# haberdashPI/SignalOperators.jl

Hardware: AMD Instinct MI355X
Metric: frames/sec sink() 44.1kHz 8ch Mix+Filt+Resample; achieved HBM GB/s (higher is better)
Workload: dtype f64

## Files before the change

signaloperators.jl_amd/csrc/executor.cpp:

```cpp
#include "plan_impl.h"

namespace so {

static inline int carrier_vec_ok(const DCarrier& c, int64_t V) {
    if (!std::getenv("SIGOPS_STRICT_ALIGN")) return (uintptr_t)c.base % (c.dtype == SO_F64 ? 8 : 4) == 0;
    return ((uintptr_t)c.base % 16 == 0) && (c.cstride % V == 0);
}

static hipError_t h2d_small(void* dst, const void* src, size_t bytes) {
    constexpr size_t kPiece = 16 * 1024;
    if (bytes < 2 * kPiece || bytes > (1u << 20)) return hipMemcpy(dst, src, bytes, hipMemcpyHostToDevice);
    for (size_t off = 0; off < bytes; off += kPiece) {
        const hipError_t e = hipMemcpy((char*)dst + off, (const char*)src + off, std::min(kPiece, bytes - off), hipMemcpyHostToDevice);
        if (e != hipSuccess) return e;
    }
    return hipSuccess;
}

static void upload_tables(Plan* P) {
    std::vector<Buf>& bufs = P->bufs;
    auto up = [&](int buf, const auto& v, size_t at = 0) {
        HIPCHECK(h2d_small((char*)bufs[buf].d + at, v.data(), v.size() * sizeof(*v.data())));
    };
    auto alloc_up = [](auto*& d, const auto& v) {
// ... 470 lines not shown
}
static RsGlobalTables global_tables(Plan* P, const Stage& S) {
    return RsGlobalTables{(const RsCtl*)P->bufs[S.ctl_buf].d, (const DCarrier*)P->bufs[S.car_buf].d, P->d_ops, P->d_leaves};
}
static void set_rsos_fixup(RsFixup& F, Plan* P, const Stage& S, const RsosItem& I) {
    F.g = I.g;
    F.tab = I.tab;
    F.jend = I.jend;
    F.jrel = (const int*)P->bufs[S.rsos_jrel_buf].d;
    F.taps = S.rsos_taps;
    F.cf = S.groups[0];
    F.gsrc = I.gsrc;
    F.y = I.y;
}
static void arm_bad(void* words, size_t n, hipStream_t st) { HIPCHECK((hipError_t)launch_fill_u32(words, n, 0x7f7f7f7fu, st)); }

static std::vector<long long> read_trace(const long long* d_trace, size_t trace_n, hipStream_t st, long long& t0) {
    std::vector<long long> tr(trace_n);
    HIPCHECK(hipStreamSynchronize(st));
    HIPCHECK(hipMemcpy(tr.data(), d_trace, trace_n * 8, hipMemcpyDeviceToHost));
    t0 = 0;
    for (size_t i = 0; i < trace_n; ++i)
        if (tr[i] && (!t0 || tr[i] < t0)) t0 = tr[i];
    return tr;
}
static void dump_rs_trace(const long long* d_trace, size_t trace_n, const RsPeriodic& rp, hipStream_t st) {
    long long t0;
    const std::vector<long long> tr = read_trace(d_trace, trace_n, st, t0);
    for (int w = 0; w < rp.nwaves; ++w)
        for (int it = 0; it < kRsTraceIters; ++it) {
            const long long* q = &tr[((size_t)w * kRsTraceIters + it) * kRsTraceStamps];
            if (!q[0]) continue;
            std::fprintf(stderr, "[rs-trace] %s w%02d it%02d", w < rp.ncompute ? "C" : "L", w, it);
            for (int k = 0; k < kRsTraceStamps; ++k) std::fprintf(stderr, " %lld", q[k] ? q[k] - t0 : -1);
            std::fprintf(stderr, "\n");
        }
}
static void dump_rsos_trace(const long long* d_trace, size_t trace_n, const RsSos& rs, hipStream_t st) {
    long long t0;
    const std::vector<long long> tr = read_trace(d_trace, trace_n, st, t0);
    const bool counters = std::atoi(std::getenv("SIGOPS_RSOS_TRACE")) == 2;
    for (int w = 0; w < rs.nwaves; ++w)
        for (int it = 0; it < (counters ? 5 : kRsosTraceIters); ++it) {
            const long long* q = &tr[((size_t)w * kRsosTraceIters + it) * 8];
            if (counters) {
                bool any = false;
                for (int k = 0; k < 8; ++k) any = any || q[k];
                if (!any) continue;
                std::fprintf(stderr, "[rsos-count] w%02d row%d", w, it);
                for (int k = 0; k < 8; ++k) std::fprintf(stderr, " %lld", q[k] - 1);
            } else {
                if (!q[0] && !q[2]) continue;
                std::fprintf(stderr, "[rsos-trace] %s w%02d it%02d", w == 0 ? "C" : (w & 3) == 0 ? "L" : "Y", w, it);
                for (int k = 0; k < 8; ++k) std::fprintf(stderr, " %lld", q[k] ? q[k] - t0 : -1);
            }
            std::fprintf(stderr, "\n");
        }
}


static int run_pointwise(Plan* P, const Step& s, void* outp, hipStream_t st) {
    const PwStep& w = P->pw[s.idx];
    if (w.nblocks <= 0) return 0;
    static const int il_scalar = std::getenv("SIGOPS_K1_ILSCALAR") ? 1 : 0;
    OutView ov{};
    if (w.out_buf >= 0) {
        const Buf& b = P->bufs[w.out_buf];
        ov = OutView{b.d, 1, b.pitch, b.dtype, il_scalar};
    } else if (P->out.is_device) {
        ov = OutView{outp, P->out.frame_stride, P->out.chan_stride, P->out.dtype, il_scalar};
    } else {
        const Buf& b = P->bufs[P->out_stage_buf];
// ... 75 lines not shown
        RsSos rs = S.rs;
        rs.out_pitch = out.pitch;
        rs.out_f32 = P->nodes[S.node].dtype == SO_F32;
        rs.f32m = 0;
        rs.sring = 0;
        rs.mats = (const double*)P->bufs[S.rsos_mats_buf].d;
        rs.bad = poison ? (int32_t*)P->bufs[B.bad_buf].d + B.bad_off[m] : nullptr;
        rs.err = kernel_error_word(P);
        I.g = rs;
        I.tab = (const double*)P->bufs[S.rsos_tab_buf].d;
        I.jend = (const int*)P->bufs[S.rsos_jend_buf].d;
        I.y = out.d - (size_t)S.rs.store_lo * (rs.out_f32 ? 4 : 8);
        I.gsrc = global_tables(P, S);
        std::memset(&fix[m], 0, sizeof fix[m]);
        set_rsos_fixup(fix[m], P, S, I);
        maxch = std::max(maxch, (int)rs.nch);
        out_f32 = rs.out_f32;
    }
    if (B.host.size() != nm || std::memcmp(B.host.data(), items.data(), nm * sizeof(RsosItem)) != 0 ||
        std::memcmp(B.fhost.data(), fix.data(), nm * sizeof(RsFixup)) != 0) {
        B.host = items;
        B.fhost = fix;
        HIPCHECK(hipMemcpyAsync(P->bufs[B.items_buf].d, B.host.data(), nm * sizeof(RsosItem), hipMemcpyHostToDevice, st));
        HIPCHECK(hipMemcpyAsync(P->bufs[B.fix_buf].d, B.fhost.data(), nm * sizeof(RsFixup), hipMemcpyHostToDevice, st));
    }
    if (poison) arm_bad(P->bufs[B.bad_buf].d, P->bufs[B.bad_buf].bytes / 4, st);
    if (launch_rsos_batch((const RsosItem*)P->bufs[B.items_buf].d, (int)nm, B.gpm, items[0].g, st) != 0)
        fail(SO_ERR_RUNTIME, "internal: no batched one-pass IIR instantiation for this geometry");
    int nl = 1;
    if (poison) nl += launch_rsos_fixup_batch((const RsFixup*)P->bufs[B.fix_buf].d, (int)nm, maxch, out_f32, st);
    return nl;
}

static int run_sample_at(Plan* P, const Step& s, void* outp, hipStream_t st) {
    const Stage& S = P->stages[s.idx];
    const Node& N = P->nodes[S.node];
    const int xdt = P->nodes[N.kids[0]].dtype;
    const View in = stage_in(P, S, N.nch, xdt), out = stage_out(P, s.idx, outp);
    SampleAtArgs a{};
    a.x = in.d;
    a.xcs = in.pitch;
    a.xfs = S.x_fstride;
    a.N = S.in_frames;
    a.x_f32 = xdt == SO_F32;
    if (S.pos_array_node >= 0) {
// ... 51 lines not shown
    a.x = in.d;
    a.xcs = in.pitch;
    a.xfs = S.x_fstride;
    a.x_f32 = xdt == SO_F32;
    a.y = (double*)out.d;
    a.ycs = out.pitch;
    a.n = S.need;
    a.nch = N.nch;
    a.tot_pitch = cumsum_totals(S.need);
    a.tot = S.aux_buf >= 0 ? (double*)P->bufs[S.aux_buf].d : nullptr;
    const int nl = launch_cumsum(a, st);
    if (nl < 0) fail(SO_ERR_UNSUPPORTED, "Cumsum: more than 65535 channels, or 2^31 chunks of 16384 frames and more, are not lowered");
    return nl;
}

static int run_rsos_fused(Plan* P, const Stage& S, const SosGeom& g, const View& out, hipStream_t st) {
    const Node& N = P->nodes[S.node];
    const Stage& S3 = P->stages[S.rsos_src];
    RsSos rs = S.rs;
    rs.out_pitch = out.pitch;
    rs.out_f32 = g.out_dtype == SO_F32 || N.dtype == SO_F32;
    if (rs.f32m && rs.out_f32) rs.ring32 = 1;
    else rs.f32m = 0;
    rs.sring = rs.f32m && (rs.fuse == 1 || rs.fuse == 2) && !std::getenv("SIGOPS_RSOS_NO_SRING") ? 1 : 0;
    char* const yk = out.d - (size_t)S.rs.store_lo * (rs.out_f32 ? 4 : 8);
    rs.store_lo = S.rs.store_lo + g.store_lo;
    rs.mats = (const double*)P->bufs[S.rsos_mats_buf].d;
    rs.bad = nullptr;
    if (S.bad_buf >= 0 && rs.nranges >= 1 && !std::getenv("SIGOPS_SOS_NOPOISON")) {
        rs.bad = (int32_t*)P->bufs[S.bad_buf].d;
        arm_bad(rs.bad, (size_t)N.nch, st);
    }
    rs.err = kernel_error_word(P);
    static long long* d_rtrace = nullptr;
    static int rtrace_seen = 0;
    const char* const rtrace_skip = std::getenv("SIGOPS_RSOS_TRACE_SKIP");
    const bool rtracing = std::getenv("SIGOPS_RSOS_TRACE") != nullptr && rtrace_seen++ >= (rtrace_skip ? std::atoi(rtrace_skip) : 0);
    const size_t rtrace_n = (size_t)16 * kRsosTraceIters * 8;
    if (rtracing) {
        if (!d_rtrace) HIPCHECK(hipMalloc(&d_rtrace, rtrace_n * 8));
        HIPCHECK(hipMemsetAsync(d_rtrace, 0, rtrace_n * 8, st));
        rs.trace = d_rtrace;
    }
    const double* rtab = (const double*)P->bufs[S.rsos_tab_buf >= 0 ? S.rsos_tab_buf : S3.tab_buf].d;
    const int* rjend = (const int*)P->bufs[S.rsos_jend_buf >= 0 ? S.rsos_jend_buf : S3.jend_buf].d;
    if (launch_rsos(rtab, rjend, rs, yk, global_tables(P, S3), S.rsos_grid, st) != 0)
        fail(SO_ERR_RUNTIME, "internal: no fused resampler + IIR instantiation for this geometry");
    if (rtracing) dump_rsos_trace(d_rtrace, rtrace_n, rs, st);
    int nl = 1;
    if (rs.bad && S.rsos_jrel_buf >= 0 && !std::getenv("SIGOPS_RSOS_NO_FIXUP")) {
        RsFixup fx{};
        set_rsos_fixup(fx, P, S, RsosItem{rs, rtab, rjend, yk, global_tables(P, S3)});
        nl += launch_rsos_fixup(fx, st);
    } else if (rs.bad) {
        SosGeom pg = g;
        pg.n = rs.n_out;
        pg.chunk = rs.pr * rs.L;
        pg.nchunks = rs.nranges;
        pg.store_lo = rs.store_lo;
        pg.bad = rs.bad;
        nl += launch_sos_poison(yk, pg, st);
    }
    return nl;
}

static int run_sos(Plan* P, const Step& s, void* outp, hipStream_t st) {
    const Stage& S = P->stages[s.idx];
    const Node& N = P->nodes[S.node];
    const size_t esz = dsize(N.dtype);
    const View in = stage_in(P, S, N.nch, N.dtype), out = stage_out(P, s.idx, outp);
    SosGeom g = S.sg;
    g.in_pitch = in.pitch;
    g.out_pitch = out.pitch;
    g.store_lo = s.idx == P->alias_stage ? P->alias_skip : 0;
    if (s.idx == P->alias_stage && P->alias_narrow) g.out_dtype = SO_F32;
    g.align_rows = S.pre_stage < 0 && !std::getenv("SIGOPS_SOS_NOALIGN");
    g.bad = nullptr;
    if (S.rsos_src >= 0) return run_rsos_fused(P, S, g, out, st);
    if (S.bad_buf >= 0 && S.pre_stage < 0 && !S.onepass && !S.xscan && !g.exact && !std::getenv("SIGOPS_SOS_NOPOISON")) {
        g.bad = (int32_t*)P->bufs[S.bad_buf].d;
        arm_bad(g.bad, (size_t)N.nch, st);
    }
// ... 500 lines not shown
```

signaloperators.jl_amd/csrc/k_exact.hip:

```cpp
#include "kcommon.h"
#include "kstage.h"

namespace so {

constexpr int kFixThreads = 256;
constexpr int kFixSeg = 1024;
constexpr int kFixIn = 6144;
constexpr int kFixAhead = 64;

template <typename TO>
__device__ __forceinline__ void rsos_fixup_body(const RsFixup& fx) {
    const RsSos& g = fx.g;
    const int ch = blockIdx.y;
    if (ch >= g.nch) return;
    const int r = g.bad[ch];
    if (r < 0 || r >= g.nranges) return;
    TO* const y = (TO*)fx.y + (int64_t)ch * g.out_pitch;
    const int64_t prL = g.pr * g.L;
    const double nan = __longlong_as_double(0x7ff8000000000000ll);
    {
        int64_t f0 = (int64_t)(r + 1) * prL;
        if (f0 < g.store_lo) f0 = g.store_lo;
        for (int64_t f = f0 + (int64_t)blockIdx.x * kFixThreads + threadIdx.x; f < g.n_out; f += (int64_t)gridDim.x * kFixThreads) y[f] = (TO)nan;
    }
    if (blockIdx.x != 0) return;
    __shared__ long long s_first;
    __shared__ double xin[kFixIn];
    __shared__ double xs[kFixSeg];
    __shared__ double ys[kFixAhead + 16];
    const int tid = threadIdx.x;
    const int64_t lo = max((int64_t)r * prL, g.store_lo), hi = min((int64_t)(r + 1) * prL, g.n_out);
// ... 64 lines not shown
                    if (!isfinite(v) || (sizeof(TO) == 4 && !isfinite((double)(float)v))) {
                        s_bad = m;
                        break;
                    }
                    ys[m - bs] = v;
                }
            }
        }
        __syncthreads();
        if (s_bad >= 0) break;
        seg = se;
    }
    const int64_t mb = s_bad;
    if (mb < 0) return;
    for (int64_t m = max(bs, lo) + tid; m < mb; m += kFixThreads) y[m] = (TO)ys[m - bs];
}

template <typename TO>
__global__ __launch_bounds__(kFixThreads) void k_rsos_fixup(RsFixup fx) {
    rsos_fixup_body<TO>(fx);
}
template <typename TO>
__global__ __launch_bounds__(kFixThreads) void k_rsos_fixup_batch(const RsFixup* __restrict__ items) {
    const RsFixup* fx = items + blockIdx.z;
    const int ch = blockIdx.y;
    if (ch >= fx->g.nch) return;
    const int r = fx->g.bad[ch];
    if (r < 0 || r >= fx->g.nranges) return;
    const RsFixup F = *fx;
    rsos_fixup_body<TO>(F);
// ... 73 lines not shown
```

signaloperators.jl_amd/csrc/k_rsos.hip:

```cpp
#include "kcommon.h"
#include "kstage.h"

#ifndef SO_RSOS_ONLY_KS
#define SO_RSOS_ONLY_KS -1
#endif
#ifndef SO_RSOS_ONLY_F32
#define SO_RSOS_ONLY_F32 0
#endif
#ifndef SO_RSOS_ONLY_NW
#define SO_RSOS_ONLY_NW 0
#endif

namespace so {

typedef double v4d __attribute__((ext_vector_type(4)));
typedef float v4f __attribute__((ext_vector_type(4)));

#define SO_LDS __attribute__((address_space(3)))
__device__ __forceinline__ int flag_ld(uint32_t a) { return *(const volatile SO_LDS int*)(uintptr_t)a; }
__device__ __forceinline__ void flag_st(uint32_t a, int v) { *(volatile SO_LDS int*)(uintptr_t)a = v; }
#define SO_SPIN_PAUSE(spins, sleep, limit)                         \
    do {                                                           \
        if (++(spins) > (limit)) rsos_wait_failed(sh);             \
        if ((sleep) == 1) __builtin_amdgcn_s_sleep(1);             \
// ... 215 lines not shown
    uint32_t SO_GLB* const e = (uint32_t SO_GLB*)rfl64((int64_t)(uintptr_t)sh->g.err);
    if (e == nullptr) __builtin_trap();
    if ((threadIdx.x & 63) == 0) __hip_atomic_store((uint32_t*)e, 1u, __ATOMIC_RELAXED, __HIP_MEMORY_SCOPE_SYSTEM);
    __threadfence_system();
    asm volatile("s_waitcnt vmcnt(0) lgkmcnt(0)" ::: "memory");
    __builtin_amdgcn_endpgm();
}

#ifndef SO_RSOS_TRACE
#define SO_RSOS_TRACE 0
#endif
__device__ __forceinline__ void rsos_stamp(long long* trace, int wave, int it, int k, int it0 = 400) {
    if constexpr (!SO_RSOS_TRACE) return;
    if (trace != nullptr && blockIdx.x == 0 && (threadIdx.x & 63) == 0 && it >= it0 && it < it0 + kRsosTraceIters)
        ((long long SO_GLB*)trace)[(wave * kRsosTraceIters + (it - it0)) * 8 + k] = clock64();
}

#ifndef SO_RSOS_COUNT
#define SO_RSOS_COUNT 0
#endif
__device__ __forceinline__ void rsos_count_out(long long* trace, int wave, int row, int k, long long v) {
    if constexpr (!SO_RSOS_COUNT) return;
    if (trace != nullptr && blockIdx.x == 0) ((long long SO_GLB*)trace)[((wave * kRsosTraceIters) + row) * 8 + k] = v + 1;
}

struct RsosLds {
    SO_LDS double *taps, *ring, *gtab;
    volatile SO_LDS double *xs, *ss;
    volatile SO_LDS double* xh;
};
// ... 682 lines not shown
        if (issued >= NK) break;
        SO_SPIN_PAUSE(spins, 2, 1 << 22);
        if constexpr (SO_RSOS_COUNT) ++cnt_idle;
    }
    __builtin_amdgcn_s_setprio(0);
    if constexpr (SO_RSOS_COUNT) {
        if (lane == 0) {
            rsos_count_out(trace, wave, 0, 0, cnt_idle);
            rsos_count_out(trace, wave, 0, 4, clock64() - cyc0);
        }
    }
}

typedef double v2d_a8 __attribute__((ext_vector_type(2), aligned(8)));

__device__ __forceinline__ bool rsos_wproj_group(const RsosShared& sh, int64_t G) {
    const RsSos& g = sh.g;
    const DCarrier& C0 = sh.ctl.car[0];
    if (!g.wproj || g.src32 || g.arr2 || g.fuse < -1 || g.ct < 8) return false;
    if (!(C0.base != nullptr && C0.vec_ok && C0.dtype == SO_F64) || (C0.df & 1)) return false;
    const int64_t ncg = g.nch / g.ct;
    const int64_t r0 = (G / ncg) * g.rgs, r1 = r0 + g.rgs - 1;
    if (r1 >= g.nranges || r0 * g.pr < g.wp) return false;
    if (g.store_lo > r0 * g.pr * g.L) return false;
    const int64_t lo_ok = C0.a > 0 ? C0.a : 0, hi_ok = C0.b < g.n_in ? C0.b : g.n_in;
    const int64_t f0 = (r0 * g.pr - g.wp) * g.M + g.wj0, f1 = (r1 * g.pr - g.wp) * g.M + g.wj0 + g.wk;
    return f0 >= lo_ok && f1 <= hi_ok;
}

template <int NY>
__device__ __attribute__((noinline)) void rsos_wproj_y(RsosShared* sh_, double* dyn, int64_t G_, int yi_) {
    constexpr int NX = 2 * NY + 1;
    const int lane = threadIdx.x & 63;
    SO_LDS RsosShared* const sh = (SO_LDS RsosShared*)rsos_lds_ptr(sh_);
    const int64_t G = rfl64(G_);
    const int yi = uni(yi_);
    const SO_LDS RsSos& g = sh->g;
    const RsosLds l = rsos_carve(dyn, uni(g.cyc) > 0 ? 0 : uni(g.ngroups) * uni(g.ks) * 64, uni(g.rpitch), NX, rsos_nss(NY));
    const uint32_t fl_base = (uint32_t)(uintptr_t)sh->flags;
    const int ct = uni(g.ct), K = uni(g.wk);
    const int npairs = (K + 7) >> 3;
    const int c0 = (int)((int64_t)yi * npairs / NY), c1 = (int)((int64_t)(yi + 1) * npairs / NY);
    const double SO_GLB* const V = (const double SO_GLB*)rfl64((int64_t)(uintptr_t)g.mats) + 14 * 64 + lane;
    const SO_LDS DCarrier& C0 = sh->ctl.car[0];
    const int64_t ncg = uni(g.nch) / ct;
    const int gq = lane >> 4, n16 = lane & 15;
    const int64_t r = (G / ncg) * uni(g.rgs) + n16 / ct;
    const int64_t f0 = (r * rfl64(g.pr) - uni(g.wp)) * rfl64(g.M) + uni(g.wj0);
    const double SO_GLB* const row = (const double SO_GLB*)rfl64((int64_t)(uintptr_t)C0.base) +
                                     ((int64_t)((int)(G % ncg) * ct + n16 % ct) * rfl64(C0.cstride) + rfl64(C0.df) + f0 + 2 * gq);
    v4d acc = v4d{0.0, 0.0, 0.0, 0.0};
    auto mm = [&](const double (&a)[16], const v2d (&b)[8]) __attribute__((always_inline)) {
#pragma unroll
        for (int i = 0; i < 8; ++i) {
            acc = __builtin_amdgcn_mfma_f64_16x16x4f64(a[2 * i], b[i][0], acc, 0, 0, 0);
            acc = __builtin_amdgcn_mfma_f64_16x16x4f64(a[2 * i + 1], b[i][1], acc, 0, 0, 0);
        }
    };
    auto load = [&](int c, double (&a)[16], v2d (&b)[8]) __attribute__((always_inline)) {
        const double SO_GLB* const vp = V + (size_t)c * 128;
        const double SO_GLB* const rp = row + (size_t)c * 8;
#pragma unroll
        for (int i = 0; i < 8; ++i) {
            a[2 * i] = vp[i * 128];
            a[2 * i + 1] = vp[i * 128 + 64];
            b[i] = *(const v2d_a8 SO_GLB*)(rp + 8 * i);
        }
    };
    double aA[16], aB[16];
    v2d bA[8], bB[8];
    const int c1f = min(c1, K >> 3);
    const int nfull = c1f > c0 ? (c1f - c0) >> 3 : 0;
    if (nfull > 0) {
        load(c0, aA, bA);
        for (int n = 0; n < nfull; n += 2) {
            const int c = c0 + 8 * n;
            if (n + 1 < nfull) load(c + 8, aB, bB);
            mm(aA, bA);
            if (n + 2 < nfull) load(c + 16, aA, bA);
            if (n + 1 < nfull) mm(aB, bB);
        }
    }
    {
        const int c = c0 + 8 * nfull;
#pragma unroll
        for (int i = 0; i < 8; ++i) {
            const int cc = c + i;
            aA[2 * i] = aA[2 * i + 1] = 0.0;
            bA[i] = v2d{0.0, 0.0};
            if (cc < c1) {
                aA[2 * i] = V[(size_t)(2 * cc) * 64];
                aA[2 * i + 1] = V[(size_t)(2 * cc + 1) * 64];
                const int f = 8 * cc + 2 * gq;
                if (f + 1 < K) bA[i] = *(const v2d_a8 SO_GLB*)(row + 8 * cc);
                else if (f < K) bA[i][0] = row[8 * cc];
            }
        }
        mm(aA, bA);
    }
#pragma unroll
    for (int v = 0; v < 3; ++v) l.ss[(1 + yi) * 192 + v * 64 + lane] = acc[v];
    flag_st(fl_base + 4 * (kRsosFlagWp + yi), 1);
}

template <int NY>
__device__ __attribute__((noinline)) void rsos_wproj_chain(RsosShared* sh_, double* dyn, int64_t G_) {
    constexpr int NX = 2 * NY + 1;
    const int lane = threadIdx.x & 63;
    SO_LDS RsosShared* const sh = (SO_LDS RsosShared*)rsos_lds_ptr(sh_);
    const int64_t G = rfl64(G_);
    const SO_LDS RsSos& g = sh->g;
    const RsosLds l = rsos_carve(dyn, uni(g.cyc) > 0 ? 0 : uni(g.ngroups) * uni(g.ks) * 64, uni(g.rpitch), NX, rsos_nss(NY));
    const uint32_t fl_base = (uint32_t)(uintptr_t)sh->flags;
    const int ct = uni(g.ct), fuse = uni(g.fuse);
    const int gq = lane >> 4, n16 = lane & 15;
    double s[3] = {0.0, 0.0, 0.0};
    if (fuse >= 0) {
        const SO_LDS DCarrier& C0 = sh->ctl.car[0];
        const DLeaf leaf0 = leaf_uniform(sh_->ctl.leaves[min(kCtlLeaves - 1, max(0, uni(C0.slot_leaf[0])))]);
        const int64_t ncg = uni(g.nch) / ct;
        const int64_t r = (G / ncg) * uni(g.rgs) + n16 / ct;
        const int64_t f0 = (r * rfl64(g.pr) - uni(g.wp)) * rfl64(g.M) + uni(g.wj0);
        const double2 sc = rsos_sine_at(f0 + leaf0.df + 1, leaf0.v0, leaf0.v1, leaf0.v2, leaf0.flag);
        const double SO_GLB* const W = (const double SO_GLB*)rfl64((int64_t)(uintptr_t)g.mats) + 14 * 64 + (size_t)((uni(g.wk) + 7) >> 3) * 128;
#pragma unroll
        for (int v = 0; v < 3; ++v) {
            const double t = fma(sc.y, W[gq + 4 * v], sc.x * W[16 + gq + 4 * v]);
            s[v] = fuse == 2 ? -t : t;
        }
    }
    int spins = 0;
    for (;;) {
        const int f = lane < NY ? flag_ld(fl_base + 4 * (kRsosFlagWp + lane)) : 1;
        if (wave_min(f, NY) >= 1) break;
        SO_SPIN_PAUSE(spins, 1, 1 << 22);
    }
#pragma unroll
    for (int yi = 0; yi < NY; ++yi)
#pragma unroll
        for (int v = 0; v < 3; ++v) s[v] += l.ss[(1 + yi) * 192 + v * 64 + lane];
#pragma unroll
    for (int v = 0; v < 3; ++v) l.ss[v * 64 + lane] = s[v];
}
// ... 477 lines not shown
    const int ru = g.ct < 8 ? g.ct : 8;
    for (int64_t G = G0; G < ngrp; G += Gstep) {
        __syncthreads();
        if (threadIdx.x < kRsosFlags) sh.flags[threadIdx.x] = 0;
        if (threadIdx.x < 192) ss[threadIdx.x] = 0.0;
        if (threadIdx.x == 0) {
            const bool pj = NW != 16 && NW != 17 && rsos_wproj_group(sh, G);
            sh.proj = pj ? 1 : 0;
            sh.wpe = pj ? 0 : g.wp;
            if (pj) sh.flags[kRsosFlagSseq] = -1;
        }
        __syncthreads();
        const bool proj = sh.proj != 0;
        if (wave == 0) {
            if (!(g.debug & 64)) {
                if (proj) rsos_wproj_chain<NY>(&sh, lds_raw, G);
                const int nk = (g.debug & 131072) ? 3 : (2 * g.nsec + 3) / 4;
                if (nk <= 1) rsos_chain<NY, 1>(&sh, lds_raw, G);
                else if (nk == 2) rsos_chain<NY, 2>(&sh, lds_raw, G);
                else rsos_chain<NY, 3>(&sh, lds_raw, G);
            }
        } else if (NW == 16 && (wave == 13 || wave == 14)) {
            if (!g.gsplit || (g.debug & 256) || g.src32) continue;
            const int q = wave - 13;
            if (g.arr2) {
                if constexpr (NL == 2) {
                    if (ru == 8) rsos_loader<NY, NL, 8, false, 0, 2, true>(&sh, lds_raw, G, q);
                    else if (ru == 4) rsos_loader<NY, NL, 4, false, 0, 2, true>(&sh, lds_raw, G, q);
                    else if (ru == 2) rsos_loader<NY, NL, 2, false, 0, 2, true>(&sh, lds_raw, G, q);
                }
            } else if (ru == 2) {
                if (g.rpitch == 770) rsos_loader<NY, NL, 2, false, 770 * 8, 2>(&sh, lds_raw, G, q);
                else if (g.rpitch == 642) rsos_loader<NY, NL, 2, false, 642 * 8, 2>(&sh, lds_raw, G, q);
                else rsos_loader<NY, NL, 2, false, 0, 2>(&sh, lds_raw, G, q);
            } else if (ru == 4) {
// ... 40 lines not shown
                else if (g.rpitch == 770) rsos_loader<NY, NL, 2, false, 770 * 8>(&sh, lds_raw, G, q);
                else if (g.rpitch == 642) rsos_loader<NY, NL, 2, false, 642 * 8>(&sh, lds_raw, G, q);
                else rsos_loader<NY, NL, 2, false>(&sh, lds_raw, G, q);
                break;
            default:
                if (g.src32) rsos_loader<NY, NL, 1, true>(&sh, lds_raw, G, q);
                else rsos_loader<NY, NL, 1, false>(&sh, lds_raw, G, q);
                break;
            }
        } else if (HW && wave == 12) {
            if (g.help && !(g.debug & 128)) rsos_helper<NY>(&sh, lds_raw);
        } else if (!(g.debug & 128))
            {
            if (NW >= 16 && wave > 12) continue;
            const int yi = NW == 16 ? (wave < 4 ? wave - 1 : wave < 8 ? wave - 2 : wave < 12 ? wave - 3 : 9) : wave - (wave > 4 ? 2 : 1);
            if (proj) rsos_wproj_y<NY>(&sh, lds_raw, G, yi);
            if constexpr (sizeof(TO) == 4 && CYC > 0) {
                if (g.f32m) {
                    rsos_ywave<KS, NY, NL, TO, CYC, true, HW>(&sh, lds_raw, G, yi);
                    continue;
                }
            }
            rsos_ywave<KS, NY, NL, TO, CYC, false, HW>(&sh, lds_raw, G, yi);
        }
    }
}

template <int KS, int NW, typename TO, int CYC>
__global__ __launch_bounds__(rsos_nthreads(NW)) void k_rsos(const double* __restrict__ tab, const int* __restrict__ jend_g, RsSos g,
                                                  TO* __restrict__ y, RsGlobalTables gsrc) {
    rsos_body<KS, NW, TO, CYC>(tab, jend_g, g, y, gsrc, (int64_t)blockIdx.x, (int64_t)gridDim.x);
// ... 163 lines not shown
```

signaloperators.jl_amd/csrc/plan_impl.h:

```cpp
#pragma once
#include <hip/hip_runtime.h>

#include <algorithm>
#include <chrono>
#include <cmath>
#include <cstdio>
#include <cstdlib>
#include <cstring>
#include <map>
#include <memory>
#include <mutex>
#include <set>
#include <string>
#include <vector>

#include "kernels.h"
#include "plan.h"
#include "sigops_internal.h"

namespace so {


struct PlanError {
    int status;
// ... 95 lines not shown
    int pos_buf = -1, pos_array_node = -1, pos_pw_step = -1;
    int64_t pos_offset = 0, pos_pitch = 0;
    int64_t x_fstride = 1;
    std::vector<DCarrier> carriers;
    int car_buf = -1;
    int ctl_buf = -1;
    std::vector<SosCoefs> groups;
    SosGeom sg{};
    int mpow_buf = -1, v_buf = -1, s0_buf = -1;
    int src_op = 0;
    DLeaf src_fn{};
    bool xscan = false;
    int batch = -1;
    int xs_mats_buf = -1, sblk_buf = -1;
    int bad_buf = -1;
    std::vector<std::vector<double>> xs_mats_host;
    std::vector<std::vector<double>> mpow_host;
    size_t mpow_stride() const {
        size_t n = 0;
        for (auto& v : mpow_host) n = std::max(n, v.size());
        return n;
    }
    bool onepass = false;
    SosOne so1{};
    int one_tabs_buf = -1, one_sync_buf = -1, one_vpub_buf = -1;
    std::vector<double> one_tabs_host;
    std::vector<size_t> one_tabs_off;
    RsGeom rg{};
    int pfb_buf = -1, dpfb_buf = -1;
    std::vector<double> pfb_host, dpfb_host;
// ... 71 lines not shown
struct SosBatch {
    std::vector<int> members;
    int nsec = 0, dtype = 0;
    int desc_buf = -1;
    int bad_buf = -1;
    std::vector<int> bad_off;
    std::vector<SosDesc> host;
    int64_t total[3] = {0, 0, 0};
};

struct RsBatch {
    std::vector<int> members;
    int gpm = 1;
    int items_buf = -1, fix_buf = -1, bad_buf = -1;
    std::vector<int> bad_off;
    std::vector<RsosItem> host;
    std::vector<RsFixup> fhost;
};

constexpr int kProfExecs = 256;

struct InterpTable {
    const double* src;
    size_t ndoubles;
    int buf;
};

struct HostLeaf {
    int node;
    const void* src;
// ... 253 lines not shown
```

signaloperators.jl_amd/csrc/sigops_internal.h:

```cpp
#pragma once
#include <cstdint>

namespace so {

enum OpCode : int32_t {
    OP_CONST = 0,
    OP_LOAD = 1,
    OP_SCALAR = 2,
    OP_FUNC = 3,
    OP_RAMP = 4,
    OP_ADD = 5,
    OP_SUB = 6,
    OP_MUL = 7,
    OP_DIV = 8,
    OP_NEG = 9,
    OP_ROUND32 = 10,
    OP_STOREF = 11,
    OP_LOADF = 12
};

enum LeafMode : int32_t { LM_PLAIN = 0, LM_CYCLE = 1, LM_MIRROR = 2 };

struct DOp {
    int32_t code;
// ... 281 lines not shown
    int32_t help;
    int32_t debug;
    int32_t cyc;
    int32_t arr2;
    int32_t wproj;
    int32_t wk;
    int32_t wj0;
    int64_t out_pitch;
    int64_t store_lo;
    const double* mats;
    int32_t* bad;
    long long* trace;
    uint32_t* err;
};
constexpr int kRsosTraceIters = 96;

struct RsosItem {
    RsSos g;
    const double* tab;
    const int* jend;
    void* y;
    RsGlobalTables gsrc;
};

struct RsFixup {
    RsSos g;
    const double* tab;
    const int* jend;
    const int* jrel;
    int32_t taps;
    int32_t pad;
    SosCoefs cf;
    RsGlobalTables gsrc;
    void* y;
};

struct RsRows {
    int64_t n_in, n_out;
    int64_t L, M;
    int64_t nperiods;
    int32_t taps;
    int32_t ct, pb;
    int32_t jlo;
    int32_t tile_len;
    int32_t pitch;
    int32_t nch;
    int32_t debug;
    int32_t kw, ngroups, pbshift;
    int32_t threads;
// ... 5 lines not shown
```

signaloperators.jl_amd/csrc/stages.cpp:

```cpp
#include "plan_impl.h"

namespace so {

static int env_int(const char* name, int dflt) {
    const char* ev = std::getenv(name);
    return ev ? std::atoi(ev) : dflt;
}

using LMat = std::vector<long double>;
static LMat lmatmul(const LMat& a, const LMat& b, int D) {
    LMat c((size_t)D * D, 0.0L);
    for (int i = 0; i < D; ++i)
        for (int k = 0; k < D; ++k) {
            long double v = a[(size_t)i * D + k];
            if (v == 0.0L) continue;
            for (int j = 0; j < D; ++j) c[(size_t)i * D + j] += v * b[(size_t)k * D + j];
        }
    return c;
}
static Mat rounded(const LMat& a) {
    Mat r(a.size());
    for (size_t i = 0; i < a.size(); ++i) r[i] = (double)a[i];
    return r;
}
// ... 1939 lines not shown
                    }
                    for (int i = 0; i < 12; ++i) {
                        mt[(size_t)14 * 64 + (size_t)K8 / 4 * 64 + i] = (double)vs[i];
                        mt[(size_t)14 * 64 + (size_t)K8 / 4 * 64 + 16 + i] = (double)vc[i];
                    }
                }
                S2.rs.wproj = 1;
                S2.rs.wk = K;
                S2.rs.wj0 = j0;
                if (std::getenv("SIGOPS_DEBUG_PLAN"))
                    std::fprintf(stderr, "[sigops] k_rsos: warm-up as one product: %d frames from %d (%d k-steps instead of %lld blocks)\n", K, j0, K8 / 4,
                                 (long long)(wp * ngp));
            }
        }
        S2.rsos_mats_buf = raw_buf(S2.rsos_mats_host.size() * 8);
        if (S2.bad_buf < 0) S2.bad_buf = raw_buf((size_t)nch * 4);
        S3.fused_away = true;
        if (alt.armed) {
            alt.armed = false;
            bufs[S3.in_buf].bytes = 0;
        }
        if (std::getenv("SIGOPS_DEBUG_PLAN"))
            std::fprintf(stderr,
                         "[sigops] resampler + IIR fused (k_rsos): %lld ranges of %lld periods (+%lld warm-up), %lld groups of %d ch x %d ranges, "
                         "ks=%d ring=%d chunk=%d waves=%d cyc=%d fuse=%d/%d\n",
                         (long long)nranges, (long long)pr, (long long)wp, (long long)ngrp, ct, rgs, ks, g.ring, g.chunk, g.nwaves, g.cyc,
                         g.fuse, g.fuse_sine);
    }
}

void Plan::fuse_plain_sos() {
// ... 145 lines not shown
        if (S.kind == ST_SOS && S.rsos_src < 0 && S.carriers.size() == 1 && S.need > 0) ++candidates;
    std::vector<size_t> small;
    for (size_t i2 = 0; i2 < stages.size(); ++i2) {
        Stage& S2 = stages[i2];
        if (S2.kind != ST_SOS || S2.rsos_src >= 0 || S2.carriers.size() != 1 || S2.need <= 0 || S2.onepass || S2.sg.exact || (S2.xscan && !S2.under_norm) ||
            (S2.under_norm && S2.norm_df != 0) || S2.batch >= 0 || S2.pre_stage >= 0 || S2.base != 0 || S2.groups.size() != 1 || S2.groups[0].nsec > 6 || S2.pw_step >= 0)
            continue;
        if (candidates > 1 && (int64_t)S2.need * nodes[S2.node].nch < ((int64_t)1 << 26) && !std::getenv("SIGOPS_RSOS_MINGROUPS")) {
            small.push_back(i2);
            continue;
        }
        RsSos g{};
        double cost = 0.0;
        if (!fit(i2, 0, g, cost)) continue;
        commit(i2, g);
        if (S2.bad_buf < 0) S2.bad_buf = raw_buf((size_t)g.nch * 4);
    }
    const char* const want_s = std::getenv("SIGOPS_RSOS_BATCH");
    const int want = want_s && *want_s ? std::atoi(want_s) : -1;
    if (small.size() < 2 || want == 0) return;
    std::map<std::pair<int, int>, std::vector<size_t>> kinds;
    for (size_t i2 : small) {
        if ((int)i2 == alias_stage) continue;
        {
            const DCarrier& c0 = stages[i2].carriers[0];
            bool plain = c0.array_node >= 0 && c0.buf < 0;
            for (int k = 0; k < c0.nslots && plain; ++k)
                if (leaves[c0.slot_leaf[k]].buf >= 0) plain = false;
            if (!plain) continue;
        }
        RsSos g{};
// ... 24 lines not shown
        if (B.members.size() < 2) continue;
        const double t_batch = (double)(((int64_t)B.members.size() * gpm + cus - 1) / cus) * worst + 15.0;
        const double t_three = (nsamp < 1e8 ? 4.4e-6 * nsamp + 25.0 : 3.4e-6 * nsamp + 110.0) * (kv.first.first ? 0.9 : 1.0) * (stepped ? 1.2 : 1.0);
        if (std::getenv("SIGOPS_DEBUG_PLAN"))
            std::fprintf(stderr, "[sigops] batched single-pass IIR estimate: %zu members x %d groups, %.0f us; three passes %.0f us\n", B.members.size(), gpm,
                         t_batch, t_three);
        if (want != 1 && t_batch > t_three) continue;
        const int bi = (int)rsbatches.size();
        int off = 0;
        for (size_t m = 0; m < B.members.size(); ++m) {
            stages[B.members[m]].rsb = bi;
            commit((size_t)B.members[m], gs[m]);
            B.bad_off.push_back(off);
            off += gs[m].nch;
        }
        B.bad_buf = raw_buf((size_t)std::max(off, 1) * 4);
        B.items_buf = raw_buf(B.members.size() * sizeof(RsosItem));
        B.fix_buf = raw_buf(B.members.size() * sizeof(RsFixup));
        rsbatches.push_back(std::move(B));
    }
}

void Plan::fuse_state_passes() {
    if (!std::getenv("SIGOPS_FUSE_STATE")) return;
    for (size_t i2 = 0; i2 < stages.size(); ++i2) {
        Stage& S2 = stages[i2];
        if (S2.kind != ST_SOS || S2.onepass || S2.need <= 0 || S2.base > 0 || S2.groups.size() != 1 || S2.in_buf < 0 ||
            S2.in_array_node >= 0 || S2.in_offset != 0 || S2.pw_step >= 0 || S2.sg.nchunks <= 1)
            continue;
        int i3 = -1;
        for (size_t j = 0; j < stages.size(); ++j)
// ... 114 lines not shown
```

Before: 29.56 billion.

## Re-arm poison flags inside the fixup kernel and zero-start first window projection

The fixup kernel now resets each channel's bad-range word itself, using a per-channel atomic tick counter. This removes the separate fill launch that re-armed the poison buffer before every run. The first row group can now use the windowed projection path by treating its pre-start samples as zero, so it no longer falls back to the slower path. The change also adds per-workgroup wall-clock tracing and doubles the size of the bad buffers to hold the counters. The re-arm state lives on the host across calls, which risks going out of sync with device state, for example when graph capture is dropped.

```diff
diff --git a/signaloperators.jl_amd/csrc/executor.cpp b/signaloperators.jl_amd/csrc/executor.cpp
--- a/signaloperators.jl_amd/csrc/executor.cpp
+++ b/signaloperators.jl_amd/csrc/executor.cpp
@@ -508,6 +508,11 @@
     F.y = I.y;
 }
 static void arm_bad(void* words, size_t n, hipStream_t st) { HIPCHECK((hipError_t)launch_fill_u32(words, n, 0x7f7f7f7fu, st)); }
+static void arm_bad_once(int32_t* words, size_t n, hipStream_t st) {
+    arm_bad(words, n, st);
+    HIPCHECK((hipError_t)launch_fill_u32(words + n, n, 0u, st));
+}
+static void drop_graph(Plan* P) { P->graph_epoch = -1; }
 
 static std::vector<long long> read_trace(const long long* d_trace, size_t trace_n, hipStream_t st, long long& t0) {
     std::vector<long long> tr(trace_n);
@@ -533,6 +538,9 @@
 static void dump_rsos_trace(const long long* d_trace, size_t trace_n, const RsSos& rs, hipStream_t st) {
     long long t0;
     const std::vector<long long> tr = read_trace(d_trace, trace_n, st, t0);
+    t0 = 0;
+    for (size_t i = 0; i < (size_t)kRsosWgTrace; ++i)
+        if (tr[i] && (!t0 || tr[i] < t0)) t0 = tr[i];
     const bool counters = std::atoi(std::getenv("SIGOPS_RSOS_TRACE")) == 2;
     for (int w = 0; w < rs.nwaves; ++w)
         for (int it = 0; it < (counters ? 5 : kRsosTraceIters); ++it) {
@@ -550,6 +558,17 @@
             }
             std::fprintf(stderr, "\n");
         }
+    int khz = 0, dev = 0;
+    HIPCHECK(hipGetDevice(&dev));
+    HIPCHECK(hipDeviceGetAttribute(&khz, hipDeviceAttributeWallClockRate, dev));
+    long long w0 = 0;
+    for (size_t G = 0; kRsosWgTrace + 4 * G + 3 < trace_n; ++G)
+        if (tr[kRsosWgTrace + 4 * G] && (!w0 || tr[kRsosWgTrace + 4 * G] < w0)) w0 = tr[kRsosWgTrace + 4 * G];
+    std::fprintf(stderr, "[rsos-wg-clock] %d kHz\n", khz);
+    for (size_t G = 0; kRsosWgTrace + 4 * G + 3 < trace_n; ++G) {
+        const long long* q = &tr[kRsosWgTrace + 4 * G];
+        if (q[0]) std::fprintf(stderr, "[rsos-wg] %zu %lld %lld %lld %d\n", G, q[0] - w0, q[1] - w0, q[2] - w0, q[3] ? 1 : 0);
+    }
 }
 
 
@@ -655,6 +674,7 @@
         I.gsrc = global_tables(P, S);
         std::memset(&fix[m], 0, sizeof fix[m]);
         set_rsos_fixup(fix[m], P, S, I);
+        if (rs.bad) fix[m].tick = rs.bad + P->bufs[B.bad_buf].bytes / 8;
         maxch = std::max(maxch, (int)rs.nch);
         out_f32 = rs.out_f32;
     }
@@ -665,11 +685,15 @@
         HIPCHECK(hipMemcpyAsync(P->bufs[B.items_buf].d, B.host.data(), nm * sizeof(RsosItem), hipMemcpyHostToDevice, st));
         HIPCHECK(hipMemcpyAsync(P->bufs[B.fix_buf].d, B.fhost.data(), nm * sizeof(RsFixup), hipMemcpyHostToDevice, st));
     }
-    if (poison) arm_bad(P->bufs[B.bad_buf].d, P->bufs[B.bad_buf].bytes / 4, st);
+    if (poison && !B.bad_armed) arm_bad_once((int32_t*)P->bufs[B.bad_buf].d, P->bufs[B.bad_buf].bytes / 8, st);
+    B.bad_armed = false;
     if (launch_rsos_batch((const RsosItem*)P->bufs[B.items_buf].d, (int)nm, B.gpm, items[0].g, st) != 0)
         fail(SO_ERR_RUNTIME, "internal: no batched one-pass IIR instantiation for this geometry");
     int nl = 1;
-    if (poison) nl += launch_rsos_fixup_batch((const RsFixup*)P->bufs[B.fix_buf].d, (int)nm, maxch, out_f32, st);
+    if (poison) {
+        nl += launch_rsos_fixup_batch((const RsFixup*)P->bufs[B.fix_buf].d, (int)nm, maxch, out_f32, st);
+        B.bad_armed = true;
+    }
     return nl;
 }
 
@@ -751,7 +775,7 @@
     return nl;
 }
 
-static int run_rsos_fused(Plan* P, const Stage& S, const SosGeom& g, const View& out, hipStream_t st) {
+static int run_rsos_fused(Plan* P, Stage& S, const SosGeom& g, const View& out, hipStream_t st) {
     const Node& N = P->nodes[S.node];
     const Stage& S3 = P->stages[S.rsos_src];
     RsSos rs = S.rs;
@@ -766,16 +790,23 @@
     rs.bad = nullptr;
     if (S.bad_buf >= 0 && rs.nranges >= 1 && !std::getenv("SIGOPS_SOS_NOPOISON")) {
         rs.bad = (int32_t*)P->bufs[S.bad_buf].d;
-        arm_bad(rs.bad, (size_t)N.nch, st);
-    }
+        if (!S.bad_armed) arm_bad_once(rs.bad, (size_t)N.nch, st);
+    }
+    S.bad_armed = false;
     rs.err = kernel_error_word(P);
     static long long* d_rtrace = nullptr;
     static int rtrace_seen = 0;
     const char* const rtrace_skip = std::getenv("SIGOPS_RSOS_TRACE_SKIP");
     const bool rtracing = std::getenv("SIGOPS_RSOS_TRACE") != nullptr && rtrace_seen++ >= (rtrace_skip ? std::atoi(rtrace_skip) : 0);
-    const size_t rtrace_n = (size_t)16 * kRsosTraceIters * 8;
+    static size_t rtrace_cap = 0;
+    const size_t rtrace_n = (size_t)kRsosWgTrace + 4 * (size_t)(rs.nch / rs.ct) * (size_t)((rs.nranges + rs.rgs - 1) / rs.rgs);
     if (rtracing) {
-        if (!d_rtrace) HIPCHECK(hipMalloc(&d_rtrace, rtrace_n * 8));
+        if (rtrace_n > rtrace_cap) {
+            if (d_rtrace) HIPCHECK(hipFree(d_rtrace));
+            d_rtrace = nullptr;
+            HIPCHECK(hipMalloc(&d_rtrace, rtrace_n * 8));
+            rtrace_cap = rtrace_n;
+        }
         HIPCHECK(hipMemsetAsync(d_rtrace, 0, rtrace_n * 8, st));
         rs.trace = d_rtrace;
     }
@@ -788,8 +819,11 @@
     if (rs.bad && S.rsos_jrel_buf >= 0 && !std::getenv("SIGOPS_RSOS_NO_FIXUP")) {
         RsFixup fx{};
         set_rsos_fixup(fx, P, S, RsosItem{rs, rtab, rjend, yk, global_tables(P, S3)});
+        fx.tick = rs.bad + N.nch;
         nl += launch_rsos_fixup(fx, st);
+        S.bad_armed = true;
     } else if (rs.bad) {
+        drop_graph(P);
         SosGeom pg = g;
         pg.n = rs.n_out;
         pg.chunk = rs.pr * rs.L;
@@ -802,7 +836,7 @@
 }
 
 static int run_sos(Plan* P, const Step& s, void* outp, hipStream_t st) {
-    const Stage& S = P->stages[s.idx];
+    Stage& S = P->stages[s.idx];
     const Node& N = P->nodes[S.node];
     const size_t esz = dsize(N.dtype);
     const View in = stage_in(P, S, N.nch, N.dtype), out = stage_out(P, s.idx, outp);
diff --git a/signaloperators.jl_amd/csrc/k_exact.hip b/signaloperators.jl_amd/csrc/k_exact.hip
--- a/signaloperators.jl_amd/csrc/k_exact.hip
+++ b/signaloperators.jl_amd/csrc/k_exact.hip
@@ -9,12 +9,8 @@
 constexpr int kFixAhead = 64;
 
 template <typename TO>
-__device__ __forceinline__ void rsos_fixup_body(const RsFixup& fx) {
+__device__ __forceinline__ void rsos_fixup_channel(const RsFixup& fx, int ch, int r) {
     const RsSos& g = fx.g;
-    const int ch = blockIdx.y;
-    if (ch >= g.nch) return;
-    const int r = g.bad[ch];
-    if (r < 0 || r >= g.nranges) return;
     TO* const y = (TO*)fx.y + (int64_t)ch * g.out_pitch;
     const int64_t prL = g.pr * g.L;
     const double nan = __longlong_as_double(0x7ff8000000000000ll);
@@ -109,6 +105,24 @@
     const int64_t mb = s_bad;
     if (mb < 0) return;
     for (int64_t m = max(bs, lo) + tid; m < mb; m += kFixThreads) y[m] = (TO)ys[m - bs];
+}
+
+template <typename TO>
+__device__ __forceinline__ void rsos_fixup_body(const RsFixup& fx) {
+    const RsSos& g = fx.g;
+    const int ch = blockIdx.y;
+    if (ch >= g.nch) return;
+    const int r = g.bad[ch];
+    if (r < 0 || r >= g.nranges) return;
+    rsos_fixup_channel<TO>(fx, ch, r);
+    __syncthreads();
+    if (threadIdx.x == 0 && fx.tick != nullptr) {
+        const int t = __hip_atomic_fetch_add(fx.tick + ch, 1, __ATOMIC_ACQ_REL, __HIP_MEMORY_SCOPE_AGENT);
+        if (t == (int)gridDim.x - 1) {
+            __hip_atomic_store(g.bad + ch, 0x7f7f7f7f, __ATOMIC_RELAXED, __HIP_MEMORY_SCOPE_AGENT);
+            __hip_atomic_store(fx.tick + ch, 0, __ATOMIC_RELAXED, __HIP_MEMORY_SCOPE_AGENT);
+        }
+    }
 }
 
 template <typename TO>
diff --git a/signaloperators.jl_amd/csrc/k_rsos.hip b/signaloperators.jl_amd/csrc/k_rsos.hip
--- a/signaloperators.jl_amd/csrc/k_rsos.hip
+++ b/signaloperators.jl_amd/csrc/k_rsos.hip
@@ -253,6 +253,10 @@
     if constexpr (!SO_RSOS_TRACE) return;
     if (trace != nullptr && blockIdx.x == 0 && (threadIdx.x & 63) == 0 && it >= it0 && it < it0 + kRsosTraceIters)
         ((long long SO_GLB*)trace)[(wave * kRsosTraceIters + (it - it0)) * 8 + k] = clock64();
+}
+
+__device__ __forceinline__ void rsos_wg_stamp(long long* wgt, int k) {
+    if ((threadIdx.x & 63) == 0) ((long long SO_GLB*)wgt)[k] = (long long)wall_clock64();
 }
 
 #ifndef SO_RSOS_COUNT
@@ -965,21 +969,25 @@
 
 typedef double v2d_a8 __attribute__((ext_vector_type(2), aligned(8)));
 
+__device__ __forceinline__ bool rsos_wproj_rows(const RsSos& g, const DCarrier& C0, int64_t ra, int64_t rb) {
+    if (rb >= g.nranges || ra * g.pr < g.wp) return false;
+    if (g.store_lo > ra * g.pr * g.L) return false;
+    const int64_t lo_ok = C0.a > 0 ? C0.a : 0, hi_ok = C0.b < g.n_in ? C0.b : g.n_in;
+    const int64_t f0 = (ra * g.pr - g.wp) * g.M + g.wj0, f1 = (rb * g.pr - g.wp) * g.M + g.wj0 + g.wk;
+    return f0 >= lo_ok && f1 <= hi_ok;
+}
 __device__ __forceinline__ bool rsos_wproj_group(const RsosShared& sh, int64_t G) {
     const RsSos& g = sh.g;
     const DCarrier& C0 = sh.ctl.car[0];
     if (!g.wproj || g.src32 || g.arr2 || g.fuse < -1 || g.ct < 8) return false;
     if (!(C0.base != nullptr && C0.vec_ok && C0.dtype == SO_F64) || (C0.df & 1)) return false;
-    const int64_t ncg = g.nch / g.ct;
-    const int64_t r0 = (G / ncg) * g.rgs, r1 = r0 + g.rgs - 1;
-    if (r1 >= g.nranges || r0 * g.pr < g.wp) return false;
-    if (g.store_lo > r0 * g.pr * g.L) return false;
-    const int64_t lo_ok = C0.a > 0 ? C0.a : 0, hi_ok = C0.b < g.n_in ? C0.b : g.n_in;
-    const int64_t f0 = (r0 * g.pr - g.wp) * g.M + g.wj0, f1 = (r1 * g.pr - g.wp) * g.M + g.wj0 + g.wk;
-    return f0 >= lo_ok && f1 <= hi_ok;
-}
-
-template <int NY>
+    const int64_t r0 = (G / (g.nch / g.ct)) * g.rgs, r1 = r0 + g.rgs - 1;
+    if (r0 > 0) return rsos_wproj_rows(g, C0, r0, r1);
+    if (g.store_lo > 0 || r1 >= g.nranges || !rsos_wproj_rows(g, C0, r1 + 1, r1 + g.rgs)) return false;
+    return r1 == 0 || rsos_wproj_rows(g, C0, 1, r1);
+}
+
+template <int NY, bool RZ>
 __device__ __attribute__((noinline)) void rsos_wproj_y(RsosShared* sh_, double* dyn, int64_t G_, int yi_) {
     constexpr int NX = 2 * NY + 1;
     const int lane = threadIdx.x & 63;
@@ -1000,6 +1008,7 @@
     const int64_t f0 = (r * rfl64(g.pr) - uni(g.wp)) * rfl64(g.M) + uni(g.wj0);
     const double SO_GLB* const row = (const double SO_GLB*)rfl64((int64_t)(uintptr_t)C0.base) +
                                      ((int64_t)((int)(G % ncg) * ct + n16 % ct) * rfl64(C0.cstride) + rfl64(C0.df) + f0 + 2 * gq);
+    const bool rz = RZ && r == 0;
     v4d acc = v4d{0.0, 0.0, 0.0, 0.0};
     auto mm = [&](const double (&a)[16], const v2d (&b)[8]) __attribute__((always_inline)) {
 #pragma unroll
@@ -1015,7 +1024,8 @@
         for (int i = 0; i < 8; ++i) {
             a[2 * i] = vp[i * 128];
             a[2 * i + 1] = vp[i * 128 + 64];
-            b[i] = *(const v2d_a8 SO_GLB*)(rp + 8 * i);
+            b[i] = v2d{0.0, 0.0};
+            if (!rz) b[i] = *(const v2d_a8 SO_GLB*)(rp + 8 * i);
         }
     };
     double aA[16], aB[16];
@@ -1043,6 +1053,7 @@
                 aA[2 * i] = V[(size_t)(2 * cc) * 64];
                 aA[2 * i + 1] = V[(size_t)(2 * cc + 1) * 64];
                 const int f = 8 * cc + 2 * gq;
+                if (rz) continue;
                 if (f + 1 < K) bA[i] = *(const v2d_a8 SO_GLB*)(row + 8 * cc);
                 else if (f < K) bA[i][0] = row[8 * cc];
             }
@@ -1073,11 +1084,12 @@
         const int64_t r = (G / ncg) * uni(g.rgs) + n16 / ct;
         const int64_t f0 = (r * rfl64(g.pr) - uni(g.wp)) * rfl64(g.M) + uni(g.wj0);
         const double2 sc = rsos_sine_at(f0 + leaf0.df + 1, leaf0.v0, leaf0.v1, leaf0.v2, leaf0.flag);
+        const bool rz = r == 0;
         const double SO_GLB* const W = (const double SO_GLB*)rfl64((int64_t)(uintptr_t)g.mats) + 14 * 64 + (size_t)((uni(g.wk) + 7) >> 3) * 128;
 #pragma unroll
         for (int v = 0; v < 3; ++v) {
             const double t = fma(sc.y, W[gq + 4 * v], sc.x * W[16 + gq + 4 * v]);
-            s[v] = fuse == 2 ? -t : t;
+            s[v] = rz ? 0.0 : fuse == 2 ? -t : t;
         }
     }
     int spins = 0;
@@ -1585,11 +1597,16 @@
         const bool proj = sh.proj != 0;
         if (wave == 0) {
             if (!(g.debug & 64)) {
+                long long* const wgt = g.trace != nullptr ? g.trace + kRsosWgTrace + 4 * G : nullptr;
+                if (wgt != nullptr) rsos_wg_stamp(wgt, 0);
                 if (proj) rsos_wproj_chain<NY>(&sh, lds_raw, G);
+                if (wgt != nullptr) rsos_wg_stamp(wgt, 1);
+                if (wgt != nullptr && proj) rsos_wg_stamp(wgt, 3);
                 const int nk = (g.debug & 131072) ? 3 : (2 * g.nsec + 3) / 4;
                 if (nk <= 1) rsos_chain<NY, 1>(&sh, lds_raw, G);
                 else if (nk == 2) rsos_chain<NY, 2>(&sh, lds_raw, G);
                 else rsos_chain<NY, 3>(&sh, lds_raw, G);
+                if (wgt != nullptr) rsos_wg_stamp(wgt, 2);
             }
         } else if (NW == 16 && (wave == 13 || wave == 14)) {
             if (!g.gsplit || (g.debug & 256) || g.src32) continue;
@@ -1660,7 +1677,10 @@
             {
             if (NW >= 16 && wave > 12) continue;
             const int yi = NW == 16 ? (wave < 4 ? wave - 1 : wave < 8 ? wave - 2 : wave < 12 ? wave - 3 : 9) : wave - (wave > 4 ? 2 : 1);
-            if (proj) rsos_wproj_y<NY>(&sh, lds_raw, G, yi);
+            if (proj) {
+                if (G < ncg) rsos_wproj_y<NY, true>(&sh, lds_raw, G, yi);
+                else rsos_wproj_y<NY, false>(&sh, lds_raw, G, yi);
+            }
             if constexpr (sizeof(TO) == 4 && CYC > 0) {
                 if (g.f32m) {
                     rsos_ywave<KS, NY, NL, TO, CYC, true, HW>(&sh, lds_raw, G, yi);
diff --git a/signaloperators.jl_amd/csrc/plan_impl.h b/signaloperators.jl_amd/csrc/plan_impl.h
--- a/signaloperators.jl_amd/csrc/plan_impl.h
+++ b/signaloperators.jl_amd/csrc/plan_impl.h
@@ -133,6 +133,7 @@
     int batch = -1;
     int xs_mats_buf = -1, sblk_buf = -1;
     int bad_buf = -1;
+    bool bad_armed = false;
     std::vector<std::vector<double>> xs_mats_host;
     std::vector<std::vector<double>> mpow_host;
     size_t mpow_stride() const {
@@ -234,6 +235,7 @@
     int gpm = 1;
     int items_buf = -1, fix_buf = -1, bad_buf = -1;
     std::vector<int> bad_off;
+    bool bad_armed = false;
     std::vector<RsosItem> host;
     std::vector<RsFixup> fhost;
 };
diff --git a/signaloperators.jl_amd/csrc/sigops_internal.h b/signaloperators.jl_amd/csrc/sigops_internal.h
--- a/signaloperators.jl_amd/csrc/sigops_internal.h
+++ b/signaloperators.jl_amd/csrc/sigops_internal.h
@@ -319,6 +319,7 @@
     uint32_t* err;
 };
 constexpr int kRsosTraceIters = 96;
+constexpr int kRsosWgTrace = 16 * kRsosTraceIters * 8;
 
 struct RsosItem {
     RsSos g;
@@ -338,6 +339,7 @@
     SosCoefs cf;
     RsGlobalTables gsrc;
     void* y;
+    int32_t* tick;
 };
 
 struct RsRows {
diff --git a/signaloperators.jl_amd/csrc/stages.cpp b/signaloperators.jl_amd/csrc/stages.cpp
--- a/signaloperators.jl_amd/csrc/stages.cpp
+++ b/signaloperators.jl_amd/csrc/stages.cpp
@@ -1977,7 +1977,8 @@
             }
         }
         S2.rsos_mats_buf = raw_buf(S2.rsos_mats_host.size() * 8);
-        if (S2.bad_buf < 0) S2.bad_buf = raw_buf((size_t)nch * 4);
+        if (S2.bad_buf < 0) S2.bad_buf = raw_buf((size_t)nch * 8);
+        bufs[S2.bad_buf].bytes = std::max(bufs[S2.bad_buf].bytes, (size_t)nch * 8);
         S3.fused_away = true;
         if (alt.armed) {
             alt.armed = false;
@@ -2153,7 +2154,8 @@
         double cost = 0.0;
         if (!fit(i2, 0, g, cost)) continue;
         commit(i2, g);
-        if (S2.bad_buf < 0) S2.bad_buf = raw_buf((size_t)g.nch * 4);
+        if (S2.bad_buf < 0) S2.bad_buf = raw_buf((size_t)g.nch * 8);
+        bufs[S2.bad_buf].bytes = std::max(bufs[S2.bad_buf].bytes, (size_t)g.nch * 8);
     }
     const char* const want_s = std::getenv("SIGOPS_RSOS_BATCH");
     const int want = want_s && *want_s ? std::atoi(want_s) : -1;
@@ -2208,7 +2210,7 @@
             B.bad_off.push_back(off);
             off += gs[m].nch;
         }
-        B.bad_buf = raw_buf((size_t)std::max(off, 1) * 4);
+        B.bad_buf = raw_buf((size_t)std::max(off, 1) * 8);
         B.items_buf = raw_buf(B.members.size() * sizeof(RsosItem));
         B.fix_buf = raw_buf(B.members.size() * sizeof(RsFixup));
         rsbatches.push_back(std::move(B));
```

After: 29.66 billion (median of 6 runs). Within noise of the previous version (+0.3%).
